# honglianghe/CDNet

Measured on AMD Instinct MI355X. Metric: tiles/sec (train fwd+bwd+Adam), 256x256, higher is better.
Workload: dtype fp32

## Files before the change

### cdnet_amd/_lib.py

```python
import ctypes as C
import os

_HERE = os.path.dirname(os.path.abspath(__file__))
LIB_PATH = os.environ.get('CDNET_LIB_PATH') or os.path.join(_HERE, 'libcdnet_hip.so')

_vp, _i, _sz, _f = C.c_void_p, C.c_int, C.c_size_t, C.c_float

class WgradReduceDesc(C.Structure):
    _fields_ = [('slab', C.c_void_p), ('dw', C.c_void_p)] + [(n, C.c_int) for n in (
        'ksplit', 'npar', 'ci_blocks', 'co_blocks', 'taps', 'CI', 'CO', 'Csrc_real', 'Cin_real', 'src_coff', 'Cout', 'mode', 'block0', 'blocks')]


SIGNATURES = {
    'cdnet_abi_version': (_i, []),
    'cdnet_abi_sizeof': (_sz, [C.c_char_p]),
    'cdnet_last_error': (C.c_char_p, []),
    'cdnet_build_info': (C.c_char_p, []),
    'cdnet_spin': (_i, [_i, _vp]),
    'cdnet_box_copy': (_i, [_vp, _vp, _sz, _vp]),
    'cdnet_box_mfma': (_i, [_vp, _vp, _vp, _i, _i, _i, _vp]),
    'cdnet_ddm_codes': (_i, [_vp, _i, _i, _i, _i, _vp, _i, _i, _vp, _vp, _vp]),
    'cdnet_ddm_normalize': (_i, [_vp, _vp, _i, _i, _i, _vp, _vp]),
    'cdnet_probmaps': (_i, [_vp, _vp, _i, _i, _i, _i, _vp, _vp, _vp]),
    'cdnet_tta_boost_argmax': (_i, [_vp, _vp, _vp, _vp, _i, _i, _vp, _i, _i, _vp, _vp, _vp, _vp, _vp, _vp]),
# ... 18 lines not shown
    'cdnet_tile_postproc': (_i, [_vp, _vp, _vp, _i, _i, _i, _i, _vp, _i, _i, _i, _i, _vp, _sz] + [_vp] * 10),
    'cdnet_cc_workspace_bytes': (_sz, [_i, _i, _i]),
    'cdnet_cc_chain': (_i, [_vp, _i, _i, _i, _i, _i, _i, _vp, _sz, _vp, _vp, _vp, _vp, _vp, _vp]),
    'cdnet_mask_views_argmax': (_i, [_vp, _i, _i, _i, _vp, _i, _i, _vp, _vp, _vp]),
    'cdnet_tile_mask_postproc_workspace_bytes': (_sz, [_i, _i, _i, _i]),
    'cdnet_tile_mask_postproc': (_i, [_vp, _i, _i, _i, _i, _i, _i, _vp, _sz] + [_vp] * 8),
    'cdnet_dilate_labels': (_i, [_vp, _i, _i, _i, _i, _vp, _vp]),
    'cdnet_conv_packed_weight_elems': (_sz, [_i] * 6),
    'cdnet_pack_conv_weights': (_i, [_vp, _vp] + [_i] * 7 + [_vp]),
    'cdnet_pack_conv_weights_scaled': (_i, [_vp, _vp, _vp] + [_i] * 7 + [_vp]),
    'cdnet_pack_batch_table_bytes': (_sz, [_i]),
    'cdnet_pack_conv_weights_batch': (_i, [_vp, _i, _vp, _sz, _i, _vp]),
    'cdnet_conv_forward': (_i, [_vp, _vp]),
    'cdnet_src_materialize': (_i, [_vp, _i, _i, _i, _vp, _vp]),
    'cdnet_input_pack': (_i, [_vp, _i, _i, _i, _i, _vp, _vp]),
    'cdnet_input_pack_f32': (_i, [_vp, _i, _i, _i, _i, _vp, _vp]),
    'cdnet_bn_fold_eval': (_i, [_vp, _vp, _vp, _vp, _vp, _f, _i, _vp, _vp, _vp]),
    'cdnet_bn_finalize_train': (_i, [_vp, _i, _i, _f, _vp, _vp, _vp, _f, _f, _vp, _vp, _vp, _vp, _vp, _vp, _vp]),
    'cdnet_dam_head_forward': (_i, [_vp, _vp, _vp, _vp, _i, _i, _i, _vp, _vp, _vp, _vp]),
    'cdnet_final_conv1x1': (_i, [_vp, _vp, _vp, _i, _i, _i, _i, _vp, _vp]),
    'cdnet_bias_grad_workspace_floats': (_sz, [_i]),
    'cdnet_bias_grad': (_i, [_vp, _sz, _i, _vp, _sz, _vp, _vp]),
    'cdnet_bias_grad_f32': (_i, [_vp, _sz, _i, _vp, _sz, _vp, _vp]),
    'cdnet_final_conv1x1_backward_workspace_floats': (_sz, []),
    'cdnet_final_conv1x1_backward': (_i, [_vp, _vp, _vp, _i, _i, _i, _i, _vp, _vp, _sz, _vp, _vp, _vp]),
    'cdnet_conv_wgrad_slab_floats': (_sz, [_i] * 6),
    'cdnet_conv_backward_weight': (_i, [_vp, _i, _i, _i, _vp] + [_i] * 9 + [_vp, _vp, _i, _vp]),
    'cdnet_wgrad_reduce_desc_fill': (_i, [_i] * 9 + [_vp, _vp, _i, _i, _vp]),
    'cdnet_wgrad_reduce_batch': (_i, [_vp, _i, _i, _vp]),
    'cdnet_bn_backward_workspace_floats': (_sz, [_i]),
    'cdnet_bn_backward': (_i, [_vp, _vp, _vp, _vp, _vp, _sz, _vp, _vp, _vp]),
    'cdnet_dam_head_backward_workspace_floats': (_sz, [_i, _i, _i]),
    'cdnet_dam_head_backward': (_i, [_vp] * 7 + [_i, _i, _i, _vp, _vp, _vp, _vp, _sz, _vp, _vp]),
    'cdnet_dam_loss_workspace_floats': (_sz, [_i, _i]),
    'cdnet_dam_loss': (_i, [_vp] * 7 + [_i, _i, _i, _i, _vp, _sz, _vp, _vp, _vp, _vp, _vp]),
    'cdnet_dam_loss_classes_workspace_floats': (_sz, [_i, _i, _i]),
    'cdnet_dam_loss_classes': (_i, [_vp] * 7 + [_i, _i, _i, _i, _i, _vp, _sz, _vp, _vp, _vp, _vp, _vp]),
    'cdnet_dam_val_sums_workspace_floats': (_sz, [_i, _i]),
    'cdnet_dam_val_sums': (_i, [_vp] * 8 + [_i, _i, _i, _vp, _sz, _vp, _vp]),
    'cdnet_dam_val_sums_classes_workspace_floats': (_sz, [_i, _i, _i]),
    'cdnet_dam_val_sums_classes': (_i, [_vp] * 8 + [_i, _i, _i, _i, _vp, _sz, _vp, _vp]),
    'cdnet_adam_step': (_i, [_vp, _vp, _vp, _vp, _sz, _f, _f, _f, _f, _f, _i, _f, _vp]),
    'cdnet_moment_step': (_i, [_vp, _vp, _vp, _vp, _vp, _sz, C.c_double, C.c_double, _f, _i, _i, _f, _f, _f, _f, _i, _f, _vp]),
    'cdnet_sgd_step': (_i, [_vp, _vp, _vp, _sz, _f, _f, _f, _i, _f, _vp]),
    'cdnet_window_pack': (_i, [_vp] + [_i] * 9 + [_vp, _vp]),
    'cdnet_window_pack_f32': (_i, [_vp] + [_i] * 9 + [_vp, _vp]),
    'cdnet_window_stitch': (_i, [_vp] + [_i] * 9 + [_vp, _vp]),
    'cdnet_label_encoding_workspace_bytes': (_sz, [_i, _i, _i, _i]),
    'cdnet_label_encoding_instances_workspace_bytes': (_sz, [_i, _i, _i, _i]),
    'cdnet_label_encoding_instances': (_i, [_vp, _i, _i, _i, _i, _vp, _vp, _vp, _sz, _vp, _vp, _vp, _vp, _vp, _vp]),
    'cdnet_augment_workspace_bytes': (_sz, [_i, _i, _i]),
    'cdnet_augment_batch': (_i, [_vp, _vp, _i, _i, _vp, _vp, _sz, _vp, _vp, _vp, _i, _vp, _vp, _vp]),
    'cdnet_label_encoding': (_i, [_vp, _i, _i, _i, _i, _vp, _vp, _vp, _sz, _vp, _vp, _vp, _vp, _vp, _vp]),
}

_lib = None


class CdnetHipError(RuntimeError):
    pass


def load():
    global _lib
    if _lib is not None:
        return _lib
# ... 50 lines not shown
```

### cdnet_amd/csrc/train.hip

```cpp
#include "common.h"
#include "xform.h"

using namespace cdnet;

namespace {

__device__ __forceinline__ float bf2f(unsigned short u) { return __uint_as_float((unsigned)u << 16); }
__device__ __forceinline__ unsigned short f2bf(float f) {
    __bf16 b = (__bf16)f;
    return __builtin_bit_cast(unsigned short, b);
}
__device__ __forceinline__ float h2f(unsigned short u) { return (float)__builtin_bit_cast(_Float16, u); }
__device__ __forceinline__ float ld16(unsigned short u, bool f16) { return f16 ? h2f(u) : bf2f(u); }

union V16 {
    uint4 u;
    unsigned short h[8];
};

inline int lin_grid(size_t total, int cap = 2048) {
    size_t g = (total + 255) / 256;
    return (int)(g > (size_t)cap ? cap : (g < 1 ? 1 : g));
}

// ... 1033 lines not shown
        for (int q = 0; q < 8; ++q) gw[0][q] = fmaf(cf[0], x[q], gw[0][q]);
        if (all16) feat_from_raw8<FM>(f2, R2, c8, s_sc[1], s_sh[1], x);
        else feat8(f2, ip, c8, s_sc[1], s_sh[1], x);
#pragma unroll
        for (int j = 0; j < 9; ++j)
#pragma unroll
            for (int q = 0; q < 8; ++q) gw[1 + j][q] = fmaf(cf[1 + j], x[q], gw[1 + j][q]);
        if (all16) feat_from_raw8<FM>(f1, R1, c8, s_sc[0], s_sh[0], x);
        else feat8(f1, ip, c8, s_sc[0], s_sh[0], x);
#pragma unroll
        for (int j = 0; j < 3; ++j)
#pragma unroll
            for (int q = 0; q < 8; ++q) gw[10 + j][q] = fmaf(cf[10 + j], x[q], gw[10 + j][q]);
    }
#pragma unroll
    for (int j = 0; j < 13; ++j)
#pragma unroll
        for (int q = 0; q < 8; ++q) {
            float t = gw[j][q];
            t += __shfl_xor(t, 8); t += __shfl_xor(t, 16); t += __shfl_xor(t, 32);
            gw[j][q] = t;
        }
    if ((tid & 63) < 8) {
#pragma unroll
        for (int j = 0; j < 13; ++j)
#pragma unroll
            for (int q = 0; q < 8; ++q) s_w[tid >> 6][j][c8 + q] = gw[j][q];
    }
    __syncthreads();
    float *o = partial + (size_t)blockIdx.x * HEADW_FLOATS;
    for (int idx = tid; idx < 13 * 64; idx += 256) {
        const int row = idx / 64, cc = idx % 64;
        o[idx] = (s_w[0][row][cc] + s_w[1][row][cc]) + (s_w[2][row][cc] + s_w[3][row][cc]);
    }
}

template <int ND> struct LossLay {
    static constexpr int PW = 9, TW = 9 + ND, SS = 9 + 2 * ND, SN = 9 + 3 * ND, SP = 9 + 4 * ND, SC = 9 + 5 * ND, SUMS = SC + 6;
    static constexpr int COEF = 6 + 4 * ND;
    static constexpr int TPB = ND > 9 ? 128 : 256;
};
template <int ND> __device__ __forceinline__ int dnext(int i) { return i == ND - 1 ? 1 : i + 1; }
template <int ND> __device__ __forceinline__ int dprev(int i) { return i == 1 ? ND - 1 : i - 1; }

struct LossIn {
    const float *mask, *point, *dirn;
    const unsigned char *label, *dirlab;
    const unsigned short *point_t;
    const unsigned char *weight;
    const int *single;
    int B, P;
    int quirk0;
};

__global__ __launch_bounds__(1024) void loss_single_kernel(const unsigned char *dirlab, const unsigned char *label, int P, int nd, int *single, int *err) {
    __shared__ int s_min[16], s_max[16], s_lmax[16];
    const unsigned char *d = dirlab + (size_t)blockIdx.x * P;
    const unsigned char *l = label + (size_t)blockIdx.x * P;
    int mn = 255, mx = 0, lm = 0;
    const int tid = threadIdx.x;
    const bool vec = (P % 16 == 0) && ((reinterpret_cast<size_t>(d) | reinterpret_cast<size_t>(l)) % 16 == 0);
    if (vec) {
        const uint4 *d4 = reinterpret_cast<const uint4 *>(d), *l4 = reinterpret_cast<const uint4 *>(l);
        for (int i = tid; i < P / 16; i += 1024) {
            const uint4 dv = d4[i], lv = l4[i];
            const unsigned dw[4] = {dv.x, dv.y, dv.z, dv.w}, lw[4] = {lv.x, lv.y, lv.z, lv.w};
// ... 575 lines not shown
        if (nflat == 0) bn_bwd_window_kernel<0, true><<<nb, 256, 0, st>>>(A, kp);
        else if (nflat == 1) bn_bwd_window_kernel<1, true><<<nb, 256, 0, st>>>(A, kp);
        else bn_bwd_window_kernel<2, true><<<nb, 256, 0, st>>>(A, kp);
    } else if (flat && dz_reuse && A.mean && A.res && dz_out) {
        BnBwdArgs B = A;
        B.ngin = 1;
        B.gin[0].g = dz_out; B.gin[0].Hg = A.H; B.gin[0].Wg = A.W; B.gin[0].oy = 0; B.gin[0].ox = 0; B.gin[0].pooled = 0;
        B.gin[0].coff = 0; B.gin[0].cstride = A.C;
        B.res = nullptr; B.relu = 0; B.dz_out = nullptr;
        bn_bwd_apply_flat_kernel<1, false><<<nb, 256, 0, st>>>(B);
    } else if (flat) {
        switch (A.ngin * 2 + (A.res ? 1 : 0)) {
            case 2: bn_bwd_apply_flat_kernel<1, false><<<nb, 256, 0, st>>>(A); break;
            case 3: bn_bwd_apply_flat_kernel<1, true><<<nb, 256, 0, st>>>(A); break;
            case 4: bn_bwd_apply_flat_kernel<2, false><<<nb, 256, 0, st>>>(A); break;
            case 5: bn_bwd_apply_flat_kernel<2, true><<<nb, 256, 0, st>>>(A); break;
            case 6: bn_bwd_apply_flat_kernel<3, false><<<nb, 256, 0, st>>>(A); break;
            default: bn_bwd_apply_flat_kernel<3, true><<<nb, 256, 0, st>>>(A); break;
        }
    } else if (window32) launch_window32<true>(A, nflat, kp, nb, st);
    else if (flat32 && A.mean && A.res && dz_out && dz_reuse) {
        BnBwdArgs B = A;
        B.ngin = 1;
        B.gin[0].g = dz_out; B.gin[0].Hg = A.H; B.gin[0].Wg = A.W; B.gin[0].oy = 0; B.gin[0].ox = 0; B.gin[0].pooled = 0;
        B.gin[0].coff = 0; B.gin[0].cstride = A.C;
        B.res = nullptr; B.relu = 0; B.dz_out = nullptr;
        launch_flat32<true>(B, nb, st);
    } else if (flat32) launch_flat32<true>(A, nb, st);
    else if (f32) bn_bwd_apply_kernel<true><<<nb, 256, 0, st>>>(A);
    else bn_bwd_apply_kernel<false><<<nb, 256, 0, st>>>(A);
    return check_launch("cdnet_bn_backward");
}

static bool bn_plain_case(const BnBwdArgs &A) {
    const GradIn &g = A.gin[0];
    return A.ngin == 1 && !g.pooled && g.oy == 0 && g.ox == 0 && g.Hg == A.H && g.Wg == A.W && A.mean && A.scale && A.shift && A.invstd && !A.res &&
           A.relu == 1 && (g.cstride == 0 || g.cstride == A.C) && g.coff == 0;
}

__global__ void bn_ktab_copy_kernel(const float *scale, const float *shift, const float *mean, const float *invstd, int C, float *ktab) {
    const int c = blockIdx.x * blockDim.x + threadIdx.x;
    if (c < C) { ktab[c] = scale[c]; ktab[C + c] = shift[c]; ktab[2 * C + c] = mean[c]; ktab[3 * C + c] = invstd[c]; }
}

extern "C" int cdnet_bn_backward_stats(const cdnet_bn_bwd_args *a, const float *gamma, float *dgamma, float *dbeta, float *workspace,
                                       size_t workspace_floats, float *ktab, void *stream) {
    BnBwdArgs A;
    int rc = fill_bn_args(a, A, "cdnet_bn_backward_stats");
    if (rc) return rc;
    CDNET_REQUIRE(bn_plain_case(A) && A.f16 != 2 && gamma && workspace && ktab, "cdnet_bn_backward_stats: plain 16-bit case only (one same-size gradient, BatchNorm + ReLU, no residual)");
    hipStream_t st = (hipStream_t)stream;
    const size_t npix = (size_t)A.N * A.H * A.W;
    CDNET_REQUIRE(npix * (size_t)A.C < ((size_t)1 << 32) && npix < ((size_t)1 << 31), "cdnet_bn_backward_stats: tensor too large for 32-bit pixel indexing");
    const int ppb = 256 / (A.C / 8);
    int nb = (int)((npix + (size_t)ppb * BN_U - 1) / ((size_t)ppb * BN_U));
    if (nb > bn_blocks_cap()) nb = bn_blocks_cap();
    if (nb < 1) nb = 1;
    const size_t need = (size_t)nb * 2 * A.C;
    if (workspace_floats < need) { set_error("cdnet_bn_backward_stats: workspace %zu < %zu floats", workspace_floats, need); return CDNET_E_WORKSPACE; }
    A.partial = workspace;
    A.draw = nullptr; A.dz_out = nullptr; A.rev = 0;
    bn_ktab_copy_kernel<<<cdiv(A.C, 256), 256, 0, st>>>(A.scale, A.shift, A.mean, A.invstd, A.C, ktab);
    bn_bwd_reduce_flat_kernel<1, false><<<nb, 256, 0, st>>>(A);
    bn_bwd_finalize_kernel<<<A.C, 256, 0, st>>>(A.partial, nb, A.C, (float)npix, gamma, A.invstd, dgamma, dbeta, ktab + 4 * A.C, ktab + 5 * A.C,
                                                 ktab + 6 * A.C);
    return check_launch("cdnet_bn_backward_stats");
}

extern "C" int cdnet_bn_backward_finalize(const cdnet_bn_bwd_args *a, const float *gamma, float *dgamma, float *dbeta, const float *partial,
                                          int nb, float *ktab, void *stream) {
    BnBwdArgs A;
    int rc = fill_bn_args(a, A, "cdnet_bn_backward_finalize");
    if (rc) return rc;
    CDNET_REQUIRE(bn_plain_case(A) && gamma && partial && ktab && nb >= 1, "cdnet_bn_backward_finalize: plain case only");
    hipStream_t st = (hipStream_t)stream;
    const size_t npix = (size_t)A.N * A.H * A.W;
    bn_bwd_finalize_kernel<<<A.C, 256, 0, st>>>(partial, nb, A.C, (float)npix, gamma, A.invstd, dgamma, dbeta, ktab + 4 * A.C, ktab + 5 * A.C,
                                                 ktab + 6 * A.C);
    return check_launch("cdnet_bn_backward_finalize");
}

extern "C" int cdnet_bn_backward_apply(const cdnet_bn_bwd_args *a, const float *ktab, uint16_t *draw, void *stream) {
    BnBwdArgs A;
    int rc = fill_bn_args(a, A, "cdnet_bn_backward_apply");
    if (rc) return rc;
    CDNET_REQUIRE(bn_plain_case(A) && ktab && draw, "cdnet_bn_backward_apply: plain case only");
    const size_t npix = (size_t)A.N * A.H * A.W;
    const bool f32 = A.f16 == 2;
    CDNET_REQUIRE(!f32 || A.C <= 1024, "cdnet_bn_backward_apply(f32): C=%d > 1024", A.C);
    const int ppb = 256 / (A.C / (f32 ? 4 : 8));
    int nb = (int)((npix + (size_t)ppb * BN_U - 1) / ((size_t)ppb * BN_U));
    if (nb > bn_blocks_cap()) nb = bn_blocks_cap();
    if (nb < 1) nb = 1;
    A.rev = 1;
    A.draw = draw; A.dz_out = nullptr;
    A.k1 = const_cast<float *>(ktab) + 4 * A.C; A.k2 = const_cast<float *>(ktab) + 5 * A.C; A.k3 = const_cast<float *>(ktab) + 6 * A.C;
    if (f32) launch_flat32<true>(A, nb, (hipStream_t)stream);
    else bn_bwd_apply_flat_kernel<1, false><<<nb, 256, 0, (hipStream_t)stream>>>(A);
    return check_launch("cdnet_bn_backward_apply");
}

extern "C" size_t cdnet_bn_backward_workspace_floats(int C) { return (size_t)BN_MAX_BLOCKS * 2 * C + 3 * (size_t)C; }

static HeadFeat mk_hf(const cdnet_head_feat &f) {
    HeadFeat h;
    h.raw = f.raw; h.res = f.res; h.scale = f.scale; h.shift = f.shift; h.relu = f.relu; h.f16 = f.f16;
    return h;
}

extern "C" int cdnet_dam_head_backward(const cdnet_head_feat *f1, const cdnet_head_feat *f2, const cdnet_head_feat *f3,
                                       const float *head_weights, const float *dmask, const float *dpoint, const float *ddir,
                                       int N, int H, int W, uint16_t *df1, uint16_t *df2, uint16_t *df3, float *workspace,
                                       size_t workspace_floats, float *dhead_weights, void *stream) {
    CDNET_REQUIRE(f1 && f2 && f3 && head_weights && dmask && dpoint && ddir && df1 && df2 && df3 && workspace && dhead_weights,
                  "cdnet_dam_head_backward: null pointer");
    static_assert(HEADW_FLOATS == CDNET_HEAD_WEIGHT_FLOATS, "head weight block");
    const size_t total = (size_t)N * H * W;
    const int nb = 1024;
    const size_t need = (size_t)nb * HEADW_FLOATS + total * 16;
    if (workspace_floats < need) { set_error("cdnet_dam_head_backward: workspace %zu < %zu floats", workspace_floats, need); return CDNET_E_WORKSPACE; }
    hipStream_t st = (hipStream_t)stream;
    float *partial = workspace, *coef = workspace + (size_t)nb * HEADW_FLOATS;
    const HeadFeat a = mk_hf(*f1), b = mk_hf(*f2), c = mk_hf(*f3);
    auto plain = [](const HeadFeat &f) { return f.f16 == 0 && !f.scale && !f.relu && !f.res; };
    auto train = [](const HeadFeat &f) { return f.f16 == 1 && f.scale && f.relu && f.res; };
    const HeadW *hw = reinterpret_cast<const HeadW *>(head_weights);
    if (plain(a) && plain(b) && plain(c)) {
        dam_head_bwd_kernel<0><<<nb, 256, 0, st>>>(a, b, c, hw, dmask, dpoint, ddir, N, H * W, df1, df2, df3, coef, partial);
        dam_head_wgrad_kernel<0><<<nb, 256, 0, st>>>(a, b, c, coef, N, H * W, partial);
    } else if (train(a) && train(b) && train(c)) {
        dam_head_bwd_kernel<1><<<nb, 256, 0, st>>>(a, b, c, hw, dmask, dpoint, ddir, N, H * W, df1, df2, df3, coef, partial);
        dam_head_wgrad_kernel<1><<<nb, 256, 0, st>>>(a, b, c, coef, N, H * W, partial);
    } else {
        dam_head_bwd_kernel<2><<<nb, 256, 0, st>>>(a, b, c, hw, dmask, dpoint, ddir, N, H * W, df1, df2, df3, coef, partial);
        dam_head_wgrad_kernel<2><<<nb, 256, 0, st>>>(a, b, c, coef, N, H * W, partial);
    }
    reduce_partials_kernel<<<cdiv(HEADW_FLOATS, 4), 256, 0, st>>>(workspace, nb, HEADW_FLOATS, dhead_weights);
    return check_launch("cdnet_dam_head_backward");
}

extern "C" size_t cdnet_dam_head_backward_workspace_floats(int N, int H, int W) {
    return (size_t)1024 * HEADW_FLOATS + (size_t)N * H * W * 16;
}

static int loss_nchunk(int P, int tpb) {
    int nchunk = cdiv(P, tpb * 8);
    return nchunk > 64 ? 64 : nchunk;
}

template <int ND>
static size_t dam_loss_ws(int B, int P) {
    using Y = LossLay<ND>;
    const int nchunk = loss_nchunk(P, Y::TPB);
    return (size_t)B * nchunk * Y::SUMS + (size_t)B * Y::COEF + (size_t)B * Y::SUMS + 16 + (size_t)B;
}

template <int ND>
static int dam_loss_impl(LossIn L, int B, int P, float *workspace, float *losses, float *dmask, float *dpoint, float *ddir, hipStream_t st) {
    using Y = LossLay<ND>;
    const int nchunk = loss_nchunk(P, Y::TPB);
    float *partial = workspace;
    float *coef = partial + (size_t)B * nchunk * Y::SUMS;
    float *sums = coef + (size_t)B * Y::COEF;
    int *err = reinterpret_cast<int *>(sums + (size_t)B * Y::SUMS);
    int *single = reinterpret_cast<int *>(sums + (size_t)B * Y::SUMS + 16);
    if (hipMemsetAsync(err, 0, sizeof(int), st) != hipSuccess) return check_launch("cdnet_dam_loss(memset)");
    L.single = single;
    loss_single_kernel<<<B, 1024, 0, st>>>(L.dirlab, L.label, P, ND, single, err);
    loss_reduce_kernel<ND><<<dim3(nchunk, B), Y::TPB, 0, st>>>(L, partial);
    loss_finalize_kernel<ND><<<1, 256, 0, st>>>(partial, nchunk, B, P, sums, coef, losses, err);
    if (dmask) loss_grad_kernel<ND><<<dim3(lin_grid((size_t)P, 256), B), 256, 0, st>>>(L, coef, dmask, dpoint, ddir);
    return check_launch("cdnet_dam_loss");
}

extern "C" size_t cdnet_dam_loss_classes_workspace_floats(int B, int P, int direction_classes) {
    return direction_classes == 5 ? dam_loss_ws<5>(B, P) : direction_classes == 17 ? dam_loss_ws<17>(B, P) : dam_loss_ws<9>(B, P);
}
// ... 136 lines not shown
```

### cdnet_amd/trainer.py

```python
import ctypes as C
import os

import torch

from . import _lib, engine, optim, runtime, streams
from .allreduce import BucketReducer, bucketed_allreduce
from .engine import Src
from .optim import HEAD_PARAMS, FlatState
from .synth import synthetic_batch


class GradIn(C.Structure):
    _fields_ = [('g', C.c_void_p), ('Hg', C.c_int), ('Wg', C.c_int), ('oy', C.c_int), ('ox', C.c_int),
                ('pooled', C.c_int), ('coff', C.c_int), ('cstride', C.c_int), ('pad_', C.c_int)]


class BnBwdArgs(C.Structure):
    _fields_ = [('raw', C.c_void_p), ('res', C.c_void_p), ('scale', C.c_void_p), ('shift', C.c_void_p),
                ('mean', C.c_void_p), ('invstd', C.c_void_p), ('gin', GradIn * 3), ('ngin', C.c_int),
                ('f16', C.c_int), ('relu', C.c_int), ('N', C.c_int), ('H', C.c_int), ('W', C.c_int), ('C', C.c_int)]


_WGRAD_WGS_DEEP, _WGRAD_WGS_SHALLOW = 128, 160
_WGRAD_WGS_KQ = 128
_WGRAD_WGS_F32 = 160
_RU_1X1_SIDE = True
WGRAD_STREAM = True
_WGRAD_DEFER = 0x100
_WGRAD_DEEP_HW = 16384


class _on_stream:
    __slots__ = ('s', 'prev')

    def __init__(self, s):
        self.s = s

    def __enter__(self):
        self.prev = torch.cuda.current_stream()
        torch.cuda.set_stream(self.s)

    def __exit__(self, *exc):
        torch.cuda.set_stream(self.prev)
        return False


class _G:
    __slots__ = ('t', 'Hg', 'Wg', 'oy', 'ox', 'pooled', 'coff', 'cstride', 'event')

    def __init__(self, t, Hg, Wg, oy=0, ox=0, pooled=0, coff=0, cstride=0):
        self.t, self.Hg, self.Wg, self.oy, self.ox, self.pooled, self.coff, self.cstride = t, Hg, Wg, oy, ox, pooled, coff, cstride
        self.event = None


def _choose_ci_tiles(C_src, Cout):
    if Cout <= 32 and runtime.PRECISION != 'fp32':
        return 1
    best, best_cost = 2, None
    for ci_t in (2, 1, 4):
        CI, CO = ci_t * 32, (4 // ci_t) * 32
        cost = -(-C_src // CI) * CI * -(-Cout // CO) * CO
        if best_cost is None or cost < best_cost:
            best, best_cost = ci_t, cost
    return best


def _wgrad_wgs(beside, HW, Cout):
    if not beside:
        return 256
    if runtime.PRECISION == 'fp32':
        return _WGRAD_WGS_F32
    if Cout <= 32 and HW > 65536:
        return _WGRAD_WGS_KQ
    return _WGRAD_WGS_DEEP if HW <= _WGRAD_DEEP_HW or HW > 65536 else _WGRAD_WGS_SHALLOW


class GradTerm(C.Structure):
    _fields_ = [('g', C.c_void_p), ('cstride', C.c_int), ('coff', C.c_int)]


class Trainer:
    G = _G

    def __init__(self, model, lr=1e-3, weight_decay=1e-4, betas=(0.9, 0.99), eps=None, quirk_sample0=True,
                 world_size=1, bucket_mb=25, optimizer='adam', momentum=0.95):
        self.model = model
        self._pack_jobs = None
        self._pack_prec = None
        self._ar = None
        self.optimizer = str(optimizer).lower()
        if self.optimizer not in optim.OPTIMIZERS:
            raise ValueError('Optimizer {} not available (one of {})'.format(optimizer, ', '.join(optim.OPTIMIZERS)))
        if eps is None:
            eps = optim.RANGER_EPS if self.optimizer == 'ranger' else 1e-8
        self.lr, self.wd, self.betas, self.eps, self.momentum = lr, weight_decay, betas, eps, momentum
        self.quirk = int(quirk_sample0)
        self.world = world_size
        self.bucket = int(float(bucket_mb) * (1 << 20) // 4)
        self.flat = FlatState(model, self.optimizer)
        model._head_flat = self.flat.P[:self.flat.n_head] if self.flat.n_head == 855 else None
        self.dev = self.flat.P.device
        self._bufs = {}
        self._wss = {}
        self.losses = torch.zeros((11,), dtype=torch.float32, device=self.dev)
        self.tape = []
        self._cat_cache = {}
        self._wstream, self._events = None, {}
        self.ar_stats = None
        self._packb_pending = False
        self._packb_stream = True
        self._side_active = False
        self._rd_mb = float(os.environ.get('CDNET_WGRAD_REDUCE_MB', '300'))
        self._rd_pending, self._rd_params, self._rd_bytes, self._rd_tables = [], [], 0, {}
        self._forwards, self._bn_base = 0, 0
        if world_size > 1:
            self.sync_from_rank0()

    def sync_from_rank0(self, src=0):
        import torch.distributed as dist
        if not (dist.is_available() and dist.is_initialized()) or dist.get_world_size() == 1:
            return
        f = self.flat
        works = [dist.broadcast(t, src=src, async_op=True) for t in (f.P, f.M, f.V, f.S) if t is not None]
        meta = torch.tensor([float(f.step_count), float(self._bn_base + self._forwards)], dtype=torch.float64, device=self.dev)
        works.append(dist.broadcast(meta, src=src, async_op=True))
        bufs = [b for b in self.model.buffers() if b.is_floating_point()]
        if bufs:
            flatb = torch.cat([b.detach().reshape(-1).float() for b in bufs])
            dist.broadcast(flatb, src=src)
            off = 0
            with torch.no_grad():
                for b in bufs:
                    b.copy_(flatb[off:off + b.numel()].view(b.shape))
                    off += b.numel()
        for w in works:
            w.wait()
        f.step_count = int(meta[0].item())
        self._bn_base, self._forwards = int(meta[1].item()), 0
        self.refresh_parameters()

    def reduce_scalars(self, values):
        import torch.distributed as dist
        if self.world <= 1 or not (dist.is_available() and dist.is_initialized()):
            return values
# ... 53 lines not shown
        m.train()
        self._forwards += 1
        runtime.TAPE = self.tape
        del self.tape[:]
        try:
            out = m(x)
        finally:
            runtime.TAPE = None
        return out

    def loss_and_grads(self, mask, point, direction, label, dirlab, point_t, weight):
        B, _, H, W = mask.shape
        lib = _lib.load()
        ND = direction.shape[1]
        ws = self._ws('loss', lib.cdnet_dam_loss_classes_workspace_floats(B, H * W, ND))
        dmask = self.buf('dmask', mask.shape, torch.float32)
        dpoint = self.buf('dpoint', point.shape, torch.float32)
        ddir = self.buf('ddir', direction.shape, torch.float32)
        assert label.dtype == torch.uint8 and dirlab.dtype == torch.uint8 and weight.dtype == torch.uint8
        assert point_t.dtype == torch.float16
        _lib.call('cdnet_dam_loss_classes', _lib.ptr(mask), _lib.ptr(point), _lib.ptr(direction), _lib.ptr(label.contiguous()),
                  _lib.ptr(dirlab.contiguous()), _lib.ptr(point_t.contiguous()), _lib.ptr(weight.contiguous()), B, H, W, ND,
                  self.quirk, _lib.ptr(ws), ws.numel(), _lib.ptr(self.losses), _lib.ptr(dmask),
                  _lib.ptr(dpoint), _lib.ptr(ddir), _lib.stream_ptr())
        return dmask, dpoint, ddir

    def backward(self, dmask, dpoint, ddir):
        m = self.model
        f1, f2, f3 = m._last_feats
        N, H, W, _ = f1.x.shape
        df = [self.buf('dF%d' % k, (N, H, W, 64), runtime.act_dtype()) for k in range(3)]
        hf = [runtime.head_feat(f) for f in (f1, f2, f3)]
        dhead = self.flat.G[:self.flat.n_head]
        ws = self._ws('head', _lib.load().cdnet_dam_head_backward_workspace_floats(N, H, W))
        _lib.call('cdnet_dam_head_backward', C.byref(hf[0]), C.byref(hf[1]), C.byref(hf[2]), _lib.ptr(m.head_weight_block()),
                  _lib.ptr(dmask), _lib.ptr(dpoint), _lib.ptr(ddir), N, H, W, _lib.ptr(df[0]), _lib.ptr(df[1]),
                  _lib.ptr(df[2]), _lib.ptr(ws), ws.numel(), _lib.ptr(dhead), _lib.stream_ptr())
        self._run_tape([(getattr(f, 'grad_to', (f.x,))[0], _G(d, H, W)) for f, d in zip((f1, f2, f3), df)], None)

    def _classifier_backward(self, key, f, conv, dl):
        N, H, W, _ = f.x.shape
        K = conv.out_channels
        df = self.buf(key, (N, H, W, 64), runtime.act_dtype())
        ws = self._ws('slab', _lib.load().cdnet_final_conv1x1_backward_workspace_floats(), side=True)
        hf = runtime.head_feat(f)
        w = conv.weight.detach().reshape(K, 64)
        _lib.call('cdnet_final_conv1x1_backward', C.byref(hf), _lib.ptr(w), _lib.ptr(dl), K, N, H, W, _lib.ptr(df), _lib.ptr(ws),
                  ws.numel(), _lib.ptr(conv.weight.grad), _lib.ptr(conv.bias.grad), _lib.stream_ptr())
        return _G(df, H, W)

    def _run_tape(self, heads, params):
        grads = {}

        def add(t, g):
            grads.setdefault(id(t), []).append(g)
        for t, g in heads:
            add(t, g)
        self._overlap_begin()
        self._overlap_done(params)
        self._backward_tape(grads, add)

    def _backward_tape(self, grads, add):
        self._cat_cache = {}
        self._rd_pending, self._rd_params, self._rd_bytes = [], [], 0
        if len(self._rd_tables) > 16:
            self._rd_tables.clear()
        self._readers, self._producer, self._bn_partials = {}, {}, {}
        self._tape_pos = {id(Lt): k for k, Lt in enumerate(self.tape)}
        for Lt in self.tape:
            if isinstance(Lt, runtime.FuseNode):
                for t in Lt.saved[0]:
# ... 36 lines not shown
            self._flush_reduces()

    def _weights_done(self, params):
        if not self._rd_pending:
            self._overlap_done(params)
            return
        self._rd_params.append(params)
        if self._rd_bytes >= self._rd_mb * (1 << 20):
            self._flush_reduces()

    def _flush_reduces(self):
        if self._rd_pending:
            key = tuple(self._rd_pending)
            tab = self._rd_tables.get(key)
            if tab is None:
                lib = _lib.load()
                descs = (_lib.WgradReduceDesc * len(key))()
                b0 = 0
                for i, a in enumerate(key):
                    _lib.call('cdnet_wgrad_reduce_desc_fill', *a, b0, C.byref(descs[i]))
                    b0 += descs[i].blocks
                dev_tab = torch.frombuffer(bytearray(bytes(descs)), dtype=torch.uint8).to(self.dev)
                tab = self._rd_tables[key] = (dev_tab, len(key), b0)
            _lib.call('cdnet_wgrad_reduce_batch', _lib.ptr(tab[0]), tab[1], tab[2], _lib.stream_ptr())
        for params in self._rd_params:
            self._overlap_done(params)
        self._rd_pending, self._rd_params, self._rd_bytes = [], [], 0

    def _layer_backward(self, k, L, gl, grads, add, side):
        srcs, out, Hl, Wl = L.saved
        No, Ho, Wo, Co = out.shape
        params = (L.weight, L.bias, None if L.bn is None else L.bn.weight, None if L.bn is None else L.bn.bias)
        part = self._bn_partials.pop(id(out), None)
        if part is not None:
            assert len(gl) == 1, (L.name, len(gl))
            a, ktab = self._bn_backward_stats(L, out, gl[0], partial=part)
            g = self.buf(('draw', L.name), (No, Ho, Wo, Co), runtime.act_dtype())
            _lib.call('cdnet_bn_backward_apply', C.byref(a), _lib.ptr(ktab), _lib.ptr(g), _lib.stream_ptr())
        elif L.bn is not None or len(gl) > 1 or gl[0].pooled or gl[0].coff or (gl[0].cstride not in (0, Co)):
            g = self._bn_backward(L, out, gl, add)
        else:
            g = gl[0].t
        if side is None:
            self._weight_backward(L, srcs, g, Hl, Wl)
            self._weights_done(params)
            self._input_backward(L, srcs, g, Hl, Wl, add)
        else:
            ev = self._event(k)
            ev.record()
            beside = _RU_1X1_SIDE and L.kind == 'conv1' and isinstance(k, tuple) and getattr(L, 'needs_input_grad', True)
            if not beside:
                self._input_backward(L, srcs, g, Hl, Wl, add)
            side.wait_event(ev)
            with _on_stream(side):
                if beside:
                    ev2 = self._event(('beside', k))

                    def add_beside(tgt, g_):
                        g_.event = ev2
                        add(tgt, g_)
                    self._input_backward(L, srcs, g, Hl, Wl, add_beside)
                    ev2.record()
                self._weight_backward(L, srcs, g, Hl, Wl)
                self._weights_done(params)

    def _bn_backward_stats(self, L, out, g, partial):
        a = self._bn_args(L, out, [_G(g.t, g.Hg, g.Wg)], res=None, relu=1)
        ktab = self.buf(('ktab', L.name), (7, out.shape[3]), torch.float32)
        bn = L.bn
        _lib.call('cdnet_bn_backward_finalize', C.byref(a), _lib.ptr(bn.weight.detach()), _lib.ptr(bn.weight.grad), _lib.ptr(bn.bias.grad),
                  _lib.ptr(partial), partial.shape[0], _lib.ptr(ktab), _lib.stream_ptr())
        return a, ktab

    def _stats_fusable(self, L, srcs, H, W, N, wpb, cfgb, cin_total):
        f32 = runtime.PRECISION == 'fp32'
        if not f32 or os.environ.get('CDNET_BN_STATS_FUSE', '1') != '1' or getattr(runtime, 'DEBUG_NORELU', False):
            return None
        if L.kind != 'conv3' or L.transposed or len(srcs) != 1:
            return None
        sx = srcs[0]
        if getattr(sx, 'is_input', False) or sx.scale is None or sx.shift is None or sx.relu is not True or sx.res is not None or sx.pool \
                or tuple(sx.off) != (0, 0) or sx.x.dtype != runtime.raw_dtype() or hasattr(sx, 'grad_to') or sx.row_stride:
            return None
        if f32 and cin_total % 64:
            return None
        P = self._producer.get(id(sx.x))
        if P is None or P.bn is None or getattr(P, 'node_res', None) is not None or getattr(P, 'node_relu', True) is not True \
                or self._readers.get(id(sx.x), 0) != 1 or tuple(sx.x.shape) != (N, H, W, cin_total):
            return None
        key = ('statsfusable', L.name, N, H, W, runtime.PRECISION)
        hit = self._bufs.get(key)
        if hit is None:
            part = torch.zeros((1024, 2, cin_total), dtype=torch.float32, device=self.dev)
            gin = self.buf(('din', L.name), (N, H, W, cin_total), runtime.act_dtype())
            gdummy = self.buf(('draw', L.name), (N, H, W, L.Cout), runtime.act_dtype())
            ok = engine.conv_forward([Src(gdummy)], wpb, cin_total, cfgb, taps=L.taps, out=gin, H=H, W=W, query_ws=True,
                                     bns=(sx.x, P.scale, P.shift, P.save_mean, P.save_invstd, part))
            hit = self._bufs[key] = (part if ok else False)
        if hit is False:
            return None
        return P, hit

    def _bn_args(self, L, out, gl, res, relu):
        a = BnBwdArgs()
        a.raw = out.data_ptr()
# ... 336 lines not shown
```

### include/cdnet_hip.h

```cpp
#ifndef CDNET_HIP_H
#define CDNET_HIP_H

#include <stddef.h>
#include <stdint.h>

#ifdef __cplusplus
extern "C" {
#endif

#define CDNET_OK            0
#define CDNET_E_ARG         1
#define CDNET_E_WORKSPACE   2
#define CDNET_E_LAUNCH      3

#define CDNET_ABI_VERSION   5

int         cdnet_abi_version(void);
size_t      cdnet_abi_sizeof(const char *struct_name);
const char *cdnet_last_error(void);
const char *cdnet_build_info(void);
int         cdnet_spin(int microseconds, void *stream);
int         cdnet_box_copy(const void *src, void *dst, size_t bytes, void *stream);
int         cdnet_box_mfma(const uint32_t *seed, float *sink, unsigned long long *stamps, int workgroups, int waves_per_wg, int iters, void *stream);

// ... 154 lines not shown
    const uint16_t *g;
    int Hg, Wg;
    int oy, ox;
    int pooled;
    int coff, cstride;
    int pad_;
} cdnet_grad_in;

typedef struct cdnet_bn_bwd_args {
    const uint16_t *raw;
    const uint16_t *res;
    const float *scale, *shift;
    const float *mean, *invstd;
    cdnet_grad_in gin[3];
    int ngin;
    int f16, relu;
    int N, H, W, C;
} cdnet_bn_bwd_args;

size_t cdnet_bn_backward_workspace_floats(int C);
int cdnet_bn_backward_stats(const cdnet_bn_bwd_args *args, const float *gamma, float *dgamma, float *dbeta, float *workspace,
                            size_t workspace_floats, float *ktab, void *stream);
int cdnet_bn_backward_apply(const cdnet_bn_bwd_args *args, const float *ktab, uint16_t *draw, void *stream);
int cdnet_bn_backward_finalize(const cdnet_bn_bwd_args *args, const float *gamma, float *dgamma, float *dbeta, const float *partial,
                               int nb, float *ktab, void *stream);
int cdnet_bn_backward(const cdnet_bn_bwd_args *args, const float *gamma, float *dgamma, float *dbeta, float *workspace,
                      size_t workspace_floats, uint16_t *draw, uint16_t *dz_out, void *stream);

size_t cdnet_dam_head_backward_workspace_floats(int N, int H, int W);
int cdnet_dam_head_backward(const cdnet_head_feat *f1, const cdnet_head_feat *f2, const cdnet_head_feat *f3,
                            const float *head_weights, const float *dmask, const float *dpoint, const float *ddir,
                            int N, int H, int W, uint16_t *df1, uint16_t *df2, uint16_t *df3, float *workspace,
                            size_t workspace_floats, float *dhead_weights, void *stream);

size_t cdnet_dam_loss_workspace_floats(int B, int P);
int cdnet_dam_loss(const float *mask, const float *point, const float *direction, const uint8_t *label,
                   const uint8_t *dirlab, const uint16_t *point_target_f16, const uint8_t *weight_u8, int B, int H, int W,
                   int quirk_sample0, float *workspace, size_t workspace_floats, float *losses, float *dmask,
                   float *dpoint, float *ddir, void *stream);
size_t cdnet_dam_loss_classes_workspace_floats(int B, int P, int direction_classes);
int cdnet_dam_loss_classes(const float *mask, const float *point, const float *direction, const uint8_t *label,
                           const uint8_t *dirlab, const uint16_t *point_target_f16, const uint8_t *weight_u8, int B, int H, int W,
                           int direction_classes, int quirk_sample0, float *workspace, size_t workspace_floats, float *losses,
                           float *dmask, float *dpoint, float *ddir, void *stream);

#define CDNET_VAL_SUMS 42
size_t cdnet_dam_val_sums_workspace_floats(int B, int P);
int cdnet_dam_val_sums(const float *mask, const float *point, const float *dirn, const uint8_t *label, const uint8_t *dirlab,
                       const uint16_t *point_target_f16, const uint8_t *weight_u8, const int *dir_rank_host, int B, int H, int W,
                       float *workspace, size_t workspace_floats, float *sums, void *stream);
size_t cdnet_dam_val_sums_classes_workspace_floats(int B, int P, int direction_classes);
int cdnet_dam_val_sums_classes(const float *mask, const float *point, const float *dirn, const uint8_t *label, const uint8_t *dirlab,
                               const uint16_t *point_target_f16, const uint8_t *weight_u8, const int *dir_rank_host,
                               int direction_classes, int B, int H, int W, float *workspace, size_t workspace_floats, float *sums,
                               void *stream);

int cdnet_adam_step(float *param, const float *grad, float *exp_avg, float *exp_avg_sq, size_t n, float lr, float beta1,
                    float beta2, float eps, float weight_decay, int step, float grad_scale, void *stream);

int cdnet_moment_step(float *param, const float *grad, float *exp_avg, float *exp_avg_sq, float *slow, size_t n, double beta1,
                      double beta2, float grad_scale, int move, int rect, float decay, float step_size, float v_div, float eps,
                      int sync, float alpha, void *stream);
int cdnet_sgd_step(float *param, const float *grad, float *momentum_buffer, size_t n, float lr, float momentum, float weight_decay,
                   int step, float grad_scale, void *stream);

int cdnet_window_pack(const float *img, int C, int H, int W, int view_xform, int tile_h, int tile_w, int stride, int ny,
// ... 67 lines not shown
```

Measured before the change: 1073.

## Fuse DAM head backward with weight-grad reduction and masked ReLU for fp32

```diff
diff --git a/cdnet_amd/_lib.py b/cdnet_amd/_lib.py
--- a/cdnet_amd/_lib.py
+++ b/cdnet_amd/_lib.py
@@ -74,6 +74,10 @@
     'cdnet_bn_backward': (_i, [_vp, _vp, _vp, _vp, _vp, _sz, _vp, _vp, _vp]),
     'cdnet_dam_head_backward_workspace_floats': (_sz, [_i, _i, _i]),
     'cdnet_dam_head_backward': (_i, [_vp] * 7 + [_i, _i, _i, _vp, _vp, _vp, _vp, _sz, _vp, _vp]),
+    'cdnet_dam_head_backward_fused_blocks': (_i, []),
+    'cdnet_dam_head_backward_fused_scratch_bytes': (_i, []),
+    'cdnet_dam_head_backward_fused_workspace_floats': (_sz, []),
+    'cdnet_dam_head_backward_fused': (_i, [_vp] * 7 + [_i, _i, _i, _vp, _vp, _vp, _vp, _sz, _vp, _vp]),
     'cdnet_dam_loss_workspace_floats': (_sz, [_i, _i]),
     'cdnet_dam_loss': (_i, [_vp] * 7 + [_i, _i, _i, _i, _vp, _sz, _vp, _vp, _vp, _vp, _vp]),
     'cdnet_dam_loss_classes_workspace_floats': (_sz, [_i, _i, _i]),
diff --git a/cdnet_amd/csrc/train.hip b/cdnet_amd/csrc/train.hip
--- a/cdnet_amd/csrc/train.hip
+++ b/cdnet_amd/csrc/train.hip
@@ -1089,6 +1089,226 @@
     for (int idx = tid; idx < 13 * 64; idx += 256) {
         const int row = idx / 64, cc = idx % 64;
         o[idx] = (s_w[0][row][cc] + s_w[1][row][cc]) + (s_w[2][row][cc] + s_w[3][row][cc]);
+    }
+}
+
+constexpr int HEAD_FUSED_BLOCKS = 1024;
+constexpr int HF_ROW = 68;
+
+template <int R0>
+__device__ __forceinline__ void head_wgrad_rows(float (&gw)[7][8], const float *cfrow, const float *f3p, const float *f2p, const float *f1p) {
+    const float4 *cr = reinterpret_cast<const float4 *>(cfrow);
+    const float4 c0 = cr[0], c1 = cr[1], c2 = cr[2], c3 = cr[3];
+    const float cf[16] = {c0.x, c0.y, c0.z, c0.w, c1.x, c1.y, c1.z, c1.w, c2.x, c2.y, c2.z, c2.w, c3.x, c3.y, c3.z, c3.w};
+    float x3[8], x2[8], x1[8];
+    if (R0 == 0) ldf8(f3p, 0, x3);
+    ldf8(f2p, 0, x2);
+    if (R0 != 0) ldf8(f1p, 0, x1);
+#pragma unroll
+    for (int r = 0; r < 7; ++r) {
+        const int row = R0 + r;
+        if (row >= 13) continue;
+#pragma unroll
+        for (int k = 0; k < 8; ++k) {
+            const float x = row == 0 ? x3[k] : row < 10 ? x2[k] : x1[k];
+            gw[r][k] = fmaf(cf[row], x, gw[r][k]);
+        }
+    }
+}
+
+__global__ __launch_bounds__(512)
+void dam_head_bwd_fused_kernel(const float *__restrict__ f1, const float *__restrict__ f2, const float *__restrict__ f3,
+                               const HeadW *__restrict__ hw, const float *__restrict__ dmask, const float *__restrict__ dpoint,
+                               const float *__restrict__ ddir, int N, int plane, float *__restrict__ df1, float *__restrict__ df2,
+                               float *__restrict__ dz3, float *__restrict__ partial, float *__restrict__ sgbuf) {
+    __shared__ HeadW w;
+    __shared__ __attribute__((aligned(16))) float s_cf[128 * 16];
+    __shared__ __attribute__((aligned(16))) float s_f[3][128 * HF_ROW];
+    __shared__ float s_sg[64 * 4][12];
+    const int tid = threadIdx.x;
+    {
+        const float *src = reinterpret_cast<const float *>(hw);
+        float *dst = reinterpret_cast<float *>(&w);
+        for (int i = tid; i < HEADW_FLOATS; i += 512) dst[i] = src[i];
+    }
+    __syncthreads();
+    const unsigned total = (unsigned)N * (unsigned)plane;
+    const int q = tid & 3, slot = tid >> 2;
+    const int sh = slot >> 5, sj = slot & 31;
+    const int c8 = (tid & 7) * 8, pg = (tid & 255) >> 3, rs = tid >> 8;
+    float sgq[6];
+#pragma unroll
+    for (int j = 0; j < 6; ++j) sgq[j] = 0.f;
+    float gw[7][8];
+#pragma unroll
+    for (int j = 0; j < 7; ++j)
+#pragma unroll
+        for (int k = 0; k < 8; ++k) gw[j][k] = 0.f;
+    for (unsigned base = blockIdx.x * 32; base < total; base += 4 * 32768) {
+        const unsigned i = base + sj + sh * 32768;
+        const bool ok = i < total;
+        const unsigned ii = ok ? i : total - 1;
+        const unsigned n = ii / (unsigned)plane, p = ii - n * (unsigned)plane;
+        asm volatile("" ::: "memory");
+        float F3[16], F2[16], F1[16], v[16];
+        const unsigned e = ii * 64 + q * 16;
+        ldf8(f3, e, F3); ldf8(f3, e + 8, F3 + 8);
+        ldf8(f2, e, F2); ldf8(f2, e + 8, F2 + 8);
+        ldf8(f1, e, F1); ldf8(f1, e + 8, F1 + 8);
+        float go_m[3], go_d[9], go_p;
+#pragma unroll
+        for (int k = 0; k < 3; ++k) go_m[k] = dmask[(n * 3 + k) * plane + p];
+#pragma unroll
+        for (int k = 0; k < 9; ++k) go_d[k] = ddir[(n * 9 + k) * plane + p];
+        go_p = dpoint[n * plane + p];
+#pragma unroll
+        for (int k = 0; k < 3; ++k) go_m[k] = ok ? go_m[k] : 0.f;
+#pragma unroll
+        for (int k = 0; k < 9; ++k) go_d[k] = ok ? go_d[k] : 0.f;
+        go_p = ok ? go_p : 0.f;
+        auto stage = [&](const float *F, int k) {
+            float *dst = s_f[k] + slot * HF_ROW + q * 16;
+#pragma unroll
+            for (int h = 0; h < 4; ++h) *reinterpret_cast<float4 *>(dst + 4 * h) = make_float4(F[4 * h], F[4 * h + 1], F[4 * h + 2], F[4 * h + 3]);
+        };
+        __syncthreads();
+        const float pt = quad_sum(xf_dot16(w.wp + q * 16, F3)) + w.bp;
+        unsigned pos3 = 0;
+#pragma unroll
+        for (int j = 0; j < 16; ++j) pos3 |= F3[j] > 0.f ? 1u << j : 0u;
+        stage(F3, 0);
+        __builtin_amdgcn_sched_barrier(0);
+        const float sg1 = 1.f / (1.f + expf(-(w.a1 * pt)));
+        const float g1 = 1.f + sg1;
+        float u[9], d[9], q2 = 0.f;
+#pragma unroll
+        for (int k = 0; k < 9; ++k) {
+            u[k] = quad_sum(xf_dot16(w.wd[k] + q * 16, F2));
+            d[k] = fmaf(g1, u[k], w.bd[k]);
+            q2 = fmaf(w.a2[k], d[k], q2);
+        }
+        stage(F2, 1);
+        __builtin_amdgcn_sched_barrier(0);
+        const float sg2 = 1.f / (1.f + expf(-q2));
+        const float g2 = 1.f + sg2;
+        float dm[3], dg2 = 0.f;
+#pragma unroll
+        for (int k = 0; k < 3; ++k) {
+            const float mk = quad_sum(xf_dot16(w.wm[k] + q * 16, F1));
+            const float go = go_m[k];
+            dg2 = fmaf(go, mk, dg2);
+            dm[k] = go * g2;
+        }
+        stage(F1, 2);
+        __builtin_amdgcn_sched_barrier(0);
+        xf_axpy16(dm[0], w.wm[0] + q * 16, v, false);
+        xf_axpy16(dm[1], w.wm[1] + q * 16, v, true);
+        xf_axpy16(dm[2], w.wm[2] + q * 16, v, true);
+        if (ok) { stf8(df1, e, v); stf8(df1, e + 8, v + 8); }
+        __builtin_amdgcn_sched_barrier(0);
+        const float dq2 = dg2 * sg2 * (1.f - sg2);
+        float du[9], dd[9], dg1 = 0.f;
+#pragma unroll
+        for (int k = 0; k < 9; ++k) {
+            dd[k] = go_d[k] + dq2 * w.a2[k];
+            dg1 = fmaf(dd[k], u[k], dg1);
+            du[k] = dd[k] * g1;
+        }
+#pragma unroll
+        for (int k = 0; k < 9; ++k) xf_axpy16(du[k], w.wd[k] + q * 16, v, k != 0);
+        if (ok) { stf8(df2, e, v); stf8(df2, e + 8, v + 8); }
+        __builtin_amdgcn_sched_barrier(0);
+        const float dsg1 = dg1 * sg1 * (1.f - sg1);
+        const float dpt = go_p + dsg1 * w.a1;
+        float sx[6], sy[6];
+        {
+            float tx[24], ty[24];
+#pragma unroll
+            for (int j = 0; j < 3; ++j) { tx[j] = go_m[j]; ty[j] = 1.f; }
+#pragma unroll
+            for (int j = 0; j < 9; ++j) { tx[3 + j] = dd[j]; ty[3 + j] = 1.f; tx[14 + j] = dq2; ty[14 + j] = d[j]; }
+            tx[12] = dpt; ty[12] = 1.f; tx[13] = dsg1; ty[13] = pt; tx[23] = 0.f; ty[23] = 0.f;
+#pragma unroll
+            for (int s = 0; s < 6; ++s) {
+                sx[s] = q == 0 ? tx[4 * s] : q == 1 ? tx[4 * s + 1] : q == 2 ? tx[4 * s + 2] : tx[4 * s + 3];
+                sy[s] = q == 0 ? ty[4 * s] : q == 1 ? ty[4 * s + 1] : q == 2 ? ty[4 * s + 2] : ty[4 * s + 3];
+            }
+        }
+        if (sh < 2) {
+#pragma unroll
+            for (int s = 0; s < 6; ++s) sgq[s] = fmaf(sx[s], sy[s], sgq[s]);
+        } else {
+#pragma unroll
+            for (int s = 0; s < 6; ++s) { s_sg[tid - 256][s] = sx[s]; s_sg[tid - 256][6 + s] = sy[s]; }
+        }
+        xf_axpy16(dpt, w.wp + q * 16, v, false);
+#pragma unroll
+        for (int j = 0; j < 16; ++j) v[j] = (pos3 >> j & 1) ? v[j] : 0.f;
+        if (ok) { stf8(dz3, e, v); stf8(dz3, e + 8, v + 8); }
+        __builtin_amdgcn_sched_barrier(0);
+        {
+            float4 cf;
+            if (q == 0) cf = make_float4(dpt, du[0], du[1], du[2]);
+            else if (q == 1) cf = make_float4(du[3], du[4], du[5], du[6]);
+            else if (q == 2) cf = make_float4(du[7], du[8], dm[0], dm[1]);
+            else cf = make_float4(dm[2], 0.f, 0.f, 0.f);
+            *reinterpret_cast<float4 *>(s_cf + slot * 16 + q * 4) = cf;
+        }
+        __syncthreads();
+        if (sh < 2) {
+#pragma unroll
+            for (int s = 0; s < 6; ++s) sgq[s] = fmaf(s_sg[tid][s], s_sg[tid][6 + s], sgq[s]);
+        }
+#pragma unroll 1
+        for (int h = 0; h < 4; ++h) {
+            if (base + pg + h * 32768 < total) {
+                const int s = h * 32 + pg;
+                if (rs == 0) head_wgrad_rows<0>(gw, s_cf + s * 16, s_f[0] + s * HF_ROW + c8, s_f[1] + s * HF_ROW + c8, s_f[2] + s * HF_ROW + c8);
+                else head_wgrad_rows<7>(gw, s_cf + s * 16, s_f[0] + s * HF_ROW + c8, s_f[1] + s * HF_ROW + c8, s_f[2] + s * HF_ROW + c8);
+            }
+        }
+    }
+    if (sh < 2) {
+        float *o = sgbuf + ((size_t)((blockIdx.x >> 1) + 512 * sh) * 64 + 32 * (blockIdx.x & 1) + sj) * 24;
+#pragma unroll
+        for (int s = 0; s < 6; ++s) o[4 * s + q] = sgq[s];
+    }
+#pragma unroll
+    for (int j = 0; j < 7; ++j)
+#pragma unroll
+        for (int k = 0; k < 8; ++k) {
+            float t = gw[j][k];
+            t += __shfl_xor(t, 8); t += __shfl_xor(t, 16); t += __shfl_xor(t, 32);
+            gw[j][k] = t;
+        }
+    __syncthreads();
+    float *s_w = s_f[0];
+    if ((tid & 63) < 8) {
+#pragma unroll
+        for (int j = 0; j < 7; ++j)
+            if (rs * 7 + j < 13) {
+#pragma unroll
+                for (int k = 0; k < 8; ++k) s_w[((((tid & 255) >> 6) * 13) + rs * 7 + j) * 64 + c8 + k] = gw[j][k];
+            }
+    }
+    __syncthreads();
+    float *o = partial + (size_t)blockIdx.x * HEADW_FLOATS;
+    for (int idx = tid; idx < 13 * 64; idx += 512) o[idx] = (s_w[idx] + s_w[832 + idx]) + (s_w[2 * 832 + idx] + s_w[3 * 832 + idx]);
+}
+
+__global__ __launch_bounds__(64) void head_scalar_reduce_kernel(const float *__restrict__ sgbuf, float *__restrict__ partial) {
+    const int tid = threadIdx.x;
+    if (tid < 23) {
+        const float *sg = sgbuf + (size_t)blockIdx.x * 64 * 24;
+        float s = 0.f;
+        for (int k = 0; k < 64; ++k) s += sg[k * 24 + tid];
+        int dst;
+        if (tid < 3) dst = 832 + 10 + tid;
+        else if (tid < 12) dst = 832 + 1 + (tid - 3);
+        else if (tid == 12) dst = 832;
+        else if (tid == 13) dst = 832 + 13;
+        else dst = 832 + 14 + (tid - 14);
+        partial[(size_t)blockIdx.x * HEADW_FLOATS + dst] = s;
     }
 }
 
@@ -1730,10 +1950,10 @@
     return check_launch("cdnet_bn_backward");
 }
 
-static bool bn_plain_case(const BnBwdArgs &A) {
+static bool bn_plain_case(const BnBwdArgs &A, bool masked = false) {
     const GradIn &g = A.gin[0];
     return A.ngin == 1 && !g.pooled && g.oy == 0 && g.ox == 0 && g.Hg == A.H && g.Wg == A.W && A.mean && A.scale && A.shift && A.invstd && !A.res &&
-           A.relu == 1 && (g.cstride == 0 || g.cstride == A.C) && g.coff == 0;
+           (A.relu == 1 || (masked && A.relu == 0)) && (g.cstride == 0 || g.cstride == A.C) && g.coff == 0;
 }
 
 __global__ void bn_ktab_copy_kernel(const float *scale, const float *shift, const float *mean, const float *invstd, int C, float *ktab) {
@@ -1782,7 +2002,7 @@
     BnBwdArgs A;
     int rc = fill_bn_args(a, A, "cdnet_bn_backward_apply");
     if (rc) return rc;
-    CDNET_REQUIRE(bn_plain_case(A) && ktab && draw, "cdnet_bn_backward_apply: plain case only");
+    CDNET_REQUIRE(bn_plain_case(A, true) && ktab && draw, "cdnet_bn_backward_apply: plain case only");
     const size_t npix = (size_t)A.N * A.H * A.W;
     const bool f32 = A.f16 == 2;
     CDNET_REQUIRE(!f32 || A.C <= 1024, "cdnet_bn_backward_apply(f32): C=%d > 1024", A.C);
@@ -1841,6 +2061,39 @@
     return (size_t)1024 * HEADW_FLOATS + (size_t)N * H * W * 16;
 }
 
+extern "C" int cdnet_dam_head_backward_fused_blocks(void) { return HEAD_FUSED_BLOCKS; }
+extern "C" int cdnet_dam_head_backward_fused_scratch_bytes(void) {
+    hipFuncAttributes at;
+    if (hipFuncGetAttributes(&at, reinterpret_cast<const void *>(dam_head_bwd_fused_kernel)) != hipSuccess) return -1;
+    return (int)at.localSizeBytes;
+}
+extern "C" size_t cdnet_dam_head_backward_fused_workspace_floats(void) { return (size_t)HEAD_FUSED_BLOCKS * (HEADW_FLOATS + 64 * 24); }
+
+extern "C" int cdnet_dam_head_backward_fused(const cdnet_head_feat *f1, const cdnet_head_feat *f2, const cdnet_head_feat *f3,
+                                             const float *head_weights, const float *dmask, const float *dpoint, const float *ddir,
+                                             int N, int H, int W, float *df1, float *df2, float *dz3, float *workspace,
+                                             size_t workspace_floats, float *dhead_weights, void *stream) {
+    CDNET_REQUIRE(f1 && f2 && f3 && head_weights && dmask && dpoint && ddir && df1 && df2 && dz3 && workspace && dhead_weights,
+                  "cdnet_dam_head_backward_fused: null pointer");
+    auto plain32 = [](const cdnet_head_feat &f) { return f.raw && f.f16 == 2 && !f.scale && !f.shift && !f.relu && !f.res; };
+    CDNET_REQUIRE(plain32(*f1) && plain32(*f2) && plain32(*f3),
+                  "cdnet_dam_head_backward_fused: plain stored fp32 features only (f16 = 2, no scale / shift / relu / res)");
+    CDNET_REQUIRE(N >= 1 && H >= 1 && W >= 1, "cdnet_dam_head_backward_fused: N=%d H=%d W=%d", N, H, W);
+    CDNET_REQUIRE((size_t)N * H * W * 64 < ((size_t)1 << 32), "cdnet_dam_head_backward_fused: tensor too large for 32-bit element indexing");
+    static_assert(HEAD_FUSED_BLOCKS == 1024, "the chains of the two-kernel path: 1024 workgroups");
+    const int nb = HEAD_FUSED_BLOCKS;
+    const size_t need = (size_t)nb * (HEADW_FLOATS + 64 * 24);
+    if (workspace_floats < need) { set_error("cdnet_dam_head_backward_fused: workspace %zu < %zu floats", workspace_floats, need); return CDNET_E_WORKSPACE; }
+    hipStream_t st = (hipStream_t)stream;
+    float *partial = workspace, *sgbuf = workspace + (size_t)nb * HEADW_FLOATS;
+    auto fp = [](const cdnet_head_feat &f) { return reinterpret_cast<const float *>(f.raw); };
+    dam_head_bwd_fused_kernel<<<nb, 512, 0, st>>>(fp(*f1), fp(*f2), fp(*f3), reinterpret_cast<const HeadW *>(head_weights), dmask, dpoint, ddir,
+                                                  N, H * W, df1, df2, dz3, partial, sgbuf);
+    head_scalar_reduce_kernel<<<nb, 64, 0, st>>>(sgbuf, partial);
+    reduce_partials_kernel<<<cdiv(HEADW_FLOATS, 4), 256, 0, st>>>(workspace, nb, HEADW_FLOATS, dhead_weights);
+    return check_launch("cdnet_dam_head_backward_fused");
+}
+
 static int loss_nchunk(int P, int tpb) {
     int nchunk = cdiv(P, tpb * 8);
     return nchunk > 64 ? 64 : nchunk;
diff --git a/cdnet_amd/trainer.py b/cdnet_amd/trainer.py
--- a/cdnet_amd/trainer.py
+++ b/cdnet_amd/trainer.py
@@ -26,6 +26,7 @@
 _WGRAD_WGS_F32 = 160
 _RU_1X1_SIDE = True
 WGRAD_STREAM = True
+HEAD_BWD_FUSE = True
 _WGRAD_DEFER = 0x100
 _WGRAD_DEEP_HW = 16384
 
@@ -46,11 +47,12 @@
 
 
 class _G:
-    __slots__ = ('t', 'Hg', 'Wg', 'oy', 'ox', 'pooled', 'coff', 'cstride', 'event')
+    __slots__ = ('t', 'Hg', 'Wg', 'oy', 'ox', 'pooled', 'coff', 'cstride', 'event', 'masked')
 
     def __init__(self, t, Hg, Wg, oy=0, ox=0, pooled=0, coff=0, cstride=0):
         self.t, self.Hg, self.Wg, self.oy, self.ox, self.pooled, self.coff, self.cstride = t, Hg, Wg, oy, ox, pooled, coff, cstride
         self.event = None
+        self.masked = False
 
 
 def _choose_ci_tiles(C_src, Cout):
@@ -110,6 +112,7 @@
         self._packb_pending = False
         self._packb_stream = True
         self._side_active = False
+        self.head_fused = False
         self._rd_mb = float(os.environ.get('CDNET_WGRAD_REDUCE_MB', '300'))
         self._rd_pending, self._rd_params, self._rd_bytes, self._rd_tables = [], [], 0, {}
         self._forwards, self._bn_base = 0, 0
@@ -229,11 +232,44 @@
         df = [self.buf('dF%d' % k, (N, H, W, 64), runtime.act_dtype()) for k in range(3)]
         hf = [runtime.head_feat(f) for f in (f1, f2, f3)]
         dhead = self.flat.G[:self.flat.n_head]
+        owner = self._head_fusable(f1, f2, f3)
+        self.head_fused = owner is not None
+        if owner is not None:
+            ws = self._ws('head', _lib.load().cdnet_dam_head_backward_fused_workspace_floats())
+            _lib.call('cdnet_dam_head_backward_fused', C.byref(hf[0]), C.byref(hf[1]), C.byref(hf[2]), _lib.ptr(m.head_weight_block()),
+                      _lib.ptr(dmask), _lib.ptr(dpoint), _lib.ptr(ddir), N, H, W, _lib.ptr(df[0]), _lib.ptr(df[1]), _lib.ptr(df[2]),
+                      _lib.ptr(ws), ws.numel(), _lib.ptr(dhead), _lib.stream_ptr())
+            heads = [(f.x, _G(d, H, W)) for f, d in zip((f1, f2, f3), df)]
+            heads[2][1].masked = True
+            self._run_tape(heads, None)
+            return
         ws = self._ws('head', _lib.load().cdnet_dam_head_backward_workspace_floats(N, H, W))
         _lib.call('cdnet_dam_head_backward', C.byref(hf[0]), C.byref(hf[1]), C.byref(hf[2]), _lib.ptr(m.head_weight_block()),
                   _lib.ptr(dmask), _lib.ptr(dpoint), _lib.ptr(ddir), N, H, W, _lib.ptr(df[0]), _lib.ptr(df[1]),
                   _lib.ptr(df[2]), _lib.ptr(ws), ws.numel(), _lib.ptr(dhead), _lib.stream_ptr())
         self._run_tape([(getattr(f, 'grad_to', (f.x,))[0], _G(d, H, W)) for f, d in zip((f1, f2, f3), df)], None)
+
+    def _head_fusable(self, f1, f2, f3):
+        if not HEAD_BWD_FUSE or runtime.PRECISION != 'fp32' or getattr(self.model, 'VARIANT', None) != 'rev1':
+            return None
+        for f in (f1, f2, f3):
+            if f.x.dtype != torch.float32 or f.scale is not None or f.shift is not None or f.res is not None or f.relu or f.pool \
+                    or hasattr(f, 'grad_to') or tuple(f.off) != (0, 0) or f.C != 64:
+                return None
+        owner = None
+        for Lt in self.tape:
+            if isinstance(Lt, runtime.FuseNode):
+                if any(t.x is f3.x for t in Lt.saved[0]):
+                    return None
+                continue
+            if any(sx.x is f3.x or sx.res is f3.x for sx in Lt.saved[0]):
+                return None
+            if Lt.saved[1] is f3.x:
+                owner = getattr(Lt, 'fused_res_of', None) if Lt.kind == 'conv1' else None
+        if owner is None or owner.bn is None or getattr(owner, 'node_relu', True) != 2 or getattr(owner, 'node_res', None) is not f3.x \
+                or owner.saved[1].dtype != torch.float32 or tuple(owner.saved[1].shape) != tuple(f3.x.shape):
+            return None
+        return owner
 
     def _classifier_backward(self, key, f, conv, dl):
         N, H, W, _ = f.x.shape
@@ -336,7 +372,9 @@
         No, Ho, Wo, Co = out.shape
         params = (L.weight, L.bias, None if L.bn is None else L.bn.weight, None if L.bn is None else L.bn.bias)
         part = self._bn_partials.pop(id(out), None)
-        if part is not None:
+        if len(gl) == 1 and gl[0].masked:
+            g = self._bn_backward_masked(L, out, gl[0], add)
+        elif part is not None:
             assert len(gl) == 1, (L.name, len(gl))
             a, ktab = self._bn_backward_stats(L, out, gl[0], partial=part)
             g = self.buf(('draw', L.name), (No, Ho, Wo, Co), runtime.act_dtype())
@@ -375,6 +413,17 @@
         _lib.call('cdnet_bn_backward_finalize', C.byref(a), _lib.ptr(bn.weight.detach()), _lib.ptr(bn.weight.grad), _lib.ptr(bn.bias.grad),
                   _lib.ptr(partial), partial.shape[0], _lib.ptr(ktab), _lib.stream_ptr())
         return a, ktab
+
+    def _bn_backward_masked(self, L, out, g, add):
+        No, Ho, Wo, Co = out.shape
+        a = self._bn_args(L, out, [_G(g.t, g.Hg, g.Wg)], res=None, relu=0)
+        draw = self.buf(('draw', L.name), (No, Ho, Wo, Co), runtime.act_dtype())
+        ws = self._ws('bn', _lib.load().cdnet_bn_backward_workspace_floats(Co))
+        bn = L.bn
+        _lib.call('cdnet_bn_backward', C.byref(a), _lib.ptr(bn.weight.detach()), _lib.ptr(bn.weight.grad), _lib.ptr(bn.bias.grad),
+                  _lib.ptr(ws), ws.numel(), _lib.ptr(draw), None, _lib.stream_ptr())
+        add(L.node_res, _G(g.t, Ho, Wo))
+        return draw
 
     def _stats_fusable(self, L, srcs, H, W, N, wpb, cfgb, cin_total):
         f32 = runtime.PRECISION == 'fp32'
diff --git a/include/cdnet_hip.h b/include/cdnet_hip.h
--- a/include/cdnet_hip.h
+++ b/include/cdnet_hip.h
@@ -210,6 +210,13 @@
                             const float *head_weights, const float *dmask, const float *dpoint, const float *ddir,
                             int N, int H, int W, uint16_t *df1, uint16_t *df2, uint16_t *df3, float *workspace,
                             size_t workspace_floats, float *dhead_weights, void *stream);
+int cdnet_dam_head_backward_fused_blocks(void);
+int cdnet_dam_head_backward_fused_scratch_bytes(void);
+size_t cdnet_dam_head_backward_fused_workspace_floats(void);
+int cdnet_dam_head_backward_fused(const cdnet_head_feat *f1, const cdnet_head_feat *f2, const cdnet_head_feat *f3,
+                                  const float *head_weights, const float *dmask, const float *dpoint, const float *ddir, int N, int H,
+                                  int W, float *df1, float *df2, float *dz3, float *workspace, size_t workspace_floats,
+                                  float *dhead_weights, void *stream);
 
 size_t cdnet_dam_loss_workspace_floats(int B, int P);
 int cdnet_dam_loss(const float *mask, const float *point, const float *direction, const uint8_t *label,
```

Result: faster. 1096 (median of 6 runs) (+2.1%).
